# shibatch/rectdetect

Hardware: AMD Instinct MI355X
Metric: 1920x1080 frames/sec (higher is better)
Workload: dtype u8/i32/f32 (bit-exact integer + IEEE f32 stencil path)

## Files before the change

rectdetect_amd/csrc/rd_k_front.hip:

```cpp
#include <stdlib.h>
#include "rd_device.h"
#include "rd_kernels.h"
#include "rectdetect_hip.h"

#define RD_LUT_ATTR __device__
#include "rd_luts.h"

namespace {

using namespace rd;
using namespace rdpix;

struct P3 { float *p[3]; };
struct P3c { const float *p[3]; };
struct SrcZ { const uint8_t *p[RD_ZB_MAX]; };

inline int cdiv(int a, int b) { return (a + b - 1) / b; }
inline dim3 grid2(int iw, int ih) { return dim3(cdiv(iw, 64), cdiv(ih, 4)); }
const dim3 block2(64, 4);
inline int grid1(int n) { int g = cdiv(n, 256); return g < 1 ? 1 : g; }

__device__ __forceinline__ int lerp_lut(const unsigned short *t, int c) { return t[c >> 8] * (256 - (c & 255)) + t[(c >> 8) + 1] * (c & 255); }

__device__ __forceinline__ uint32_t plab_of(const unsigned short *s_s2l, const unsigned short *s_cf, const unsigned short *s_cf2, int b, int g, int r) {
// ... 222 lines not shown
    } else if (FMT == RD_PIX_NV12) yuv_bgr(byte(8 * sr + sx), byte(16 + 2 * j), byte(17 + 2 * j), pb, pg, pr);
    else yuv_bgr(byte(8 * sr + sx), byte(16 + j), byte(20 + j), pb, pg, pr);
    b += pb; g += pg; r += pr;
  }
  b >>= 2; g >>= 2; r >>= 2;
}

template <int FMT>
__global__ __launch_bounds__(256) void k_pix2plab_half_t(uint32_t *__restrict__ out, P3 dst, PixZ src, int iw, int ih, size_t zs) {
  const int z = blockIdx.z;
  const uint8_t *__restrict__ p0 = src.p[0][z], *__restrict__ p1 = src.p[1][z], *__restrict__ p2 = src.p[2][z];
  RD_ZSHIFT(zs, out, dst.p[0], dst.p[1], dst.p[2]);
  __shared__ unsigned short s_s2l[RD_LUT_S2L_N], s_cf[RD_LUT_CF_N], s_cf2[RD_LUT_CF_N];
  __shared__ unsigned short tile[3][64][66];
  const int tid = rd_ty() * 64 + threadIdx.x;
  const int x0 = blockIdx.x * 64, y0 = blockIdx.y * 64;
  const int cx = (tid & 15) * 4, r0 = tid >> 4;
  const int x = x0 + cx, m = min(iw - x, 4);
  uint32_t w[4][HalfW<FMT>::n] = {};
#pragma unroll
  for (int k = 0; k < 4; k++) {
    const int y = y0 + r0 + 16 * k;
    if (m > 0 && y < ih) pix_load_half<FMT>(w[k], p0, p1, p2, src.pitch, x, y, m, src.wide != 0);
  }
  for (int i = tid; i < RD_LUT_S2L_N; i += 256) s_s2l[i] = rd_lut_s2l[i];
  for (int i = tid; i < RD_LUT_CF_N; i += 256) { s_cf[i] = rd_lut_cfunc[i]; s_cf2[i] = rd_lut_cfunc2[i]; }
  __syncthreads();
#pragma unroll
  for (int k = 0; k < 4; k++) {
    const int r = r0 + 16 * k, y = y0 + r;
    if (m <= 0 || y >= ih) continue;
    uint32_t v[4];
#pragma unroll
    for (int j = 0; j < 4; j++) {
      int b, g, rr;
      pix_bgr_half<FMT>(w[k], j, b, g, rr);
      v[j] = plab_of(s_s2l, s_cf, s_cf2, b, g, rr);
      tile[0][r][cx + j] = (unsigned short)(v[j] & 4095u); tile[1][r][cx + j] = (unsigned short)((v[j] >> 12) & 1023u); tile[2][r][cx + j] = (unsigned short)((v[j] >> 22) & 1023u);
    }
    uint32_t *o = out + (size_t)y * iw + x;
    if (m == 4 && (iw & 3) == 0) *(uint4 *)o = make_uint4(v[0], v[1], v[2], v[3]);
    else for (int j = 0; j < m; j++) o[j] = v[j];
  }
  __syncthreads();
  for (int r = rd_ty(); r < 64; r += 4) {
    const int ox = y0 + threadIdx.x, oy = x0 + r;
    if (ox < ih && oy < iw)
      for (int k = 0; k < 3; k++) ((unsigned short *)dst.p[k])[(size_t)oy * ih + ox] = tile[k][threadIdx.x][r];
  }
}

template <typename LD, typename ST> __device__ __forceinline__ void ew4(int n, LD ld, ST st) {
  const int stride = gridDim.x * blockDim.x;
  int i = blockIdx.x * blockDim.x + threadIdx.x;
  for (; i + 3 * stride < n; i += 4 * stride) {
    const auto v0 = ld(i), v1 = ld(i + stride), v2 = ld(i + 2 * stride), v3 = ld(i + 3 * stride);
    st(i, v0); st(i + stride, v1); st(i + 2 * stride, v2); st(i + 3 * stride, v3);
  }
  for (; i < n; i += stride) st(i, ld(i));
}

__global__ void k_unpack_plab(float *__restrict__ L, float *__restrict__ a, float *__restrict__ b, const uint32_t *__restrict__ in, int n) {
  for (int i = blockIdx.x * blockDim.x + threadIdx.x; i < n; i += gridDim.x * blockDim.x) {
    float l, aa, bb;
    unpack_lab(in[i], l, aa, bb);
    L[i] = l; a[i] = aa; b[i] = bb;
  }
}

__global__ void k_pack_plab(uint32_t *__restrict__ out, const float *__restrict__ L, const float *__restrict__ a, const float *__restrict__ b, int n) {
  ew4(n, [=](int i) { return make_float3(L[i], a[i], b[i]); }, [=](int i, float3 v) { out[i] = pack_lab(v.x, v.y, v.z); });
}

template <int MODE>
__global__ __launch_bounds__(256) void k_transpose(P3 dst, P3c src, P3c fwd, P3c bwd, const uint32_t *__restrict__ plab, int np, int W, int H, const int *only_if) {
  if (only_if && *only_if == 0) return;
  __shared__ float tile[3][64][65];
  const int x0 = blockIdx.x * 64, y0 = blockIdx.y * 64;
  for (int r = rd_ty(); r < 64; r += 4) {
    const int x = x0 + threadIdx.x, y = y0 + r;
    if (x < W && y < H) {
      const size_t i = (size_t)y * W + x;
      if (MODE == 1) {
        float l, a, b;
        unpack_lab(plab[i], l, a, b);
        tile[0][r][threadIdx.x] = l; tile[1][r][threadIdx.x] = a; tile[2][r][threadIdx.x] = b;
      } else if (MODE == 2) {
        for (int k = 0; k < np; k++) tile[k][r][threadIdx.x] = bwd.p[k][i] + fwd.p[k][i] - src.p[k][i] * 0.3989422804f;
      } else {
        for (int k = 0; k < np; k++) tile[k][r][threadIdx.x] = src.p[k][i];
      }
    }
  }
  __syncthreads();
  for (int r = rd_ty(); r < 64; r += 4) {
    const int ox = y0 + threadIdx.x, oy = x0 + r;
    if (ox < H && oy < W)
      for (int k = 0; k < np; k++) dst.p[k][(size_t)oy * H + ox] = tile[k][threadIdx.x][r];
  }
}

#define IIR_C0 0.3989422804f
#define IIR_C1 0.1414542400f
#define IIR_C2 -0.0030406818f
#define IIR_C3 -0.0041116157f
#define IIR_C4 0.0006696623f
#define IIR_C5 0.0000498707f
#define IIR_C6 -0.0000449761f
#define IIR_C7 -0.0000051528f
#define IIR_C8 0.2519574622f
#define IIR_C9 -0.0098627835f
#define IIR_C10 -0.0067013653f
#define IIR_C11 0.0012572396f
#define IIR_C12 0.0000481394f
#define IIR_C13 -0.0000097781f
#define IIR_C14 0.0000006462f
#define IIR_WARM 11
#ifndef IIR_CH
#define IIR_CH 16
#endif

#define IF_ROWS_MIN 64
#define IF_WU 32
#define IF_PITCH 65
__host__ __device__ inline int if_nchunks(int H, int rows) {
  int n = (H + rows - 1) / rows;
  if (n > 1 && H % rows != 0 && H % rows < 8) n--;
  return n;
}

typedef float iir_f2 __attribute__((ext_vector_type(2)));
#define IIR_STATE iir_f2 q1 = 0, q2 = 0, q3 = 0, q4 = 0, q5 = 0, q6 = 0, q7 = 0
#define IIR_STEP(i0v)                                                                                                  \
  iir_f2 acc = (iir_f2){IIR_C1, IIR_C8} * q1;                                                                          \
  acc = acc + (iir_f2){IIR_C2, IIR_C9} * q2;                                                                           \
  acc = acc + (iir_f2){IIR_C3, IIR_C10} * q3;                                                                          \
  acc = acc + (iir_f2){IIR_C4, IIR_C11} * q4;                                                                          \
  acc = acc + (iir_f2){IIR_C5, IIR_C12} * q5;                                                                          \
  acc = acc + (iir_f2){IIR_C6, IIR_C13} * q6;                                                                          \
  acc = acc + (iir_f2){IIR_C7, IIR_C14} * q7;                                                                          \
  float d = (i0v) * IIR_C0;                                                                                            \
  d += acc.x;                                                                                                          \
  d += acc.y;
#define IIR_SHIFT(i0v)                                                                                                 \
  q7 = q6; q6 = q5; q5 = q4; q4 = q3; q3 = q2; q2 = q1; q1 = (iir_f2){(i0v), d};

template <int SRC16> struct iir_src { typedef float T; };
template <> struct iir_src<1> { typedef unsigned short T; };
template <int SRC16, typename T> __device__ __forceinline__ float iir_field(T v, float sc, float hf) {
  if (SRC16) return (float)(int)v * sc + hf;
  return (float)v;
}
template <int TOUT, int IF_ROWS, int SRC16>
__global__ __launch_bounds__(128) void k_iir_fused(P3 dst, P3c src, float *__restrict__ tails, int W, int H, int nchunks, int *bad, int np, size_t zs) {
  __shared__ float fwt[(IF_ROWS + 8) * IF_PITCH];
  const int lane = threadIdx.x & 63, anti = threadIdx.x >> 6;
  const int k = blockIdx.y % np, c = blockIdx.z;
  float *dk = k == 0 ? dst.p[0] : (k == 1 ? dst.p[1] : dst.p[2]);
  const float *sk = k == 0 ? src.p[0] : (k == 1 ? src.p[1] : src.p[2]);
  { const size_t rd_zoff_ = (size_t)(blockIdx.y / np) * zs; RD_ZS1(dk); RD_ZS1(sk); RD_ZS1(tails); RD_ZS1(bad); }
  if (blockIdx.x == 0 && k == 0 && blockIdx.z == 0 && threadIdx.x == 0) *bad = 0;
  const int x = blockIdx.x * 64 + lane;
  const bool xin = x < W;
  typedef typename iir_src<SRC16>::T TS;
  const TS *__restrict__ in = (const TS *)sk;
  const unsigned xs = (unsigned)(xin ? x : W - 1) * (unsigned)sizeof(TS), x4 = (unsigned)(xin ? x : W - 1) * 4u;
#define IIR_ROW(ptr) (*(const TS *)((const char *)(ptr) + xs))
#define IIR_OUT(ptr) (*(float *)((char *)(ptr) + x4))
  const float sc = k == 0 ? 1.0f / 4096 : 1.0f / 1024, hf = k == 0 ? 0.5f / 4096 : 0.5f / 1024;
#define IIR_LD(v) iir_field<SRC16>(v, sc, hf)
  const int s0 = c * IF_ROWS, s1 = (c == nchunks - 1) ? H : s0 + IF_ROWS;
  const int mid = s0 + (s1 - s0) / 2;
  float *__restrict__ tl = tails + ((size_t)(k * nchunks + c) * 4 * 7) * W;
  const int ylo = -IIR_WARM, yhi = H + IIR_WARM;
  float cur[IIR_CH], nxt[IIR_CH];
  static_assert(IIR_CH >= 8 && IF_WU % IIR_CH == 0 && (IF_ROWS / 2) % IIR_CH == 0, "the interior path walks whole chunks, half a block per phase");
  if (s0 - IF_WU >= 0 && s1 + IF_WU <= H && s1 - s0 == IF_ROWS) {
#define IIR_CHUNK(PTR, STEP, STORE, TAIL, TIDX) IIR_CHUNK_(PTR, STEP, STORE, TAIL, TIDX, 1)
#define IIR_CHUNK_(PTR, STEP, STORE, TAIL, TIDX, MORE)                                                                  \
    {                                                                                                                    \
      if (MORE) { _Pragma("unroll") for (int j = 0; j < IIR_CH; j++) nxt[j] = IIR_LD(IIR_ROW((PTR) + ((long)(IIR_CH + j) * (STEP)) * W)); } \
      _Pragma("unroll") for (int j = 0; j < IIR_CH; j++) {                                                               \
        IIR_STEP(cur[j]);                                                                                                \
        STORE;                                                                                                           \
        if ((TAIL) >= 0 && j >= IIR_CH - 7 && xin) IIR_OUT(tl + (size_t)((TAIL) * 7 + (TIDX)) * W) = d;                            \
        IIR_SHIFT(cur[j]);                                                                                               \
      }                                                                                                                  \
      _Pragma("unroll") for (int j = 0; j < IIR_CH; j++) cur[j] = nxt[j];                                                \
    }
    constexpr int HALF = IF_ROWS / 2 / IIR_CH;
    IIR_STATE;
    if (!anti) {
      const TS *p = in + (size_t)(s0 - IF_WU) * W;
#pragma unroll
      for (int j = 0; j < IIR_CH; j++) cur[j] = IIR_LD(IIR_ROW(p + (size_t)j * W));
      for (int q = 0; q < IF_WU / IIR_CH - 1; q++) { IIR_CHUNK(p, 1, (void)0, -1, 0); p += (size_t)IIR_CH * W; }
      IIR_CHUNK(p, 1, (void)0, 0, j - (IIR_CH - 7)); p += (size_t)IIR_CH * W;
      float *f = fwt + lane;
      for (int q = 0; q < HALF; q++) { IIR_CHUNK(p, 1, f[j * IF_PITCH] = d, -1, 0); p += (size_t)IIR_CH * W; f += IIR_CH * IF_PITCH; }
      __syncthreads();
      float *o = TOUT ? nullptr : dk + (size_t)mid * W;
#define IIR_FINISH_F { const float r = (f[j * IF_PITCH] + d) - cur[j] * IIR_C0; if (TOUT) f[j * IF_PITCH] = r; else if (xin) IIR_OUT(o + (long)j * W) = r; }
      for (int q = 0; q < HALF - 1; q++) { IIR_CHUNK(p, 1, IIR_FINISH_F, -1, 0); p += (size_t)IIR_CH * W; f += IIR_CH * IF_PITCH; if (!TOUT) o += (size_t)IIR_CH * W; }
      IIR_CHUNK_(p, 1, IIR_FINISH_F, 1, j - (IIR_CH - 7), 0);
#undef IIR_FINISH_F
    } else {
      const TS *p = in + (size_t)(s1 - 1 + IF_WU) * W;
#pragma unroll
      for (int j = 0; j < IIR_CH; j++) cur[j] = IIR_LD(IIR_ROW(p - (long)j * W));
      for (int q = 0; q < IF_WU / IIR_CH - 1; q++) { IIR_CHUNK(p, -1, (void)0, -1, 0); p -= (size_t)IIR_CH * W; }
      IIR_CHUNK(p, -1, (void)0, 2, (IIR_CH - 1) - j); p -= (size_t)IIR_CH * W;
      float *f = fwt + (IF_ROWS - 1) * IF_PITCH + lane;
      for (int q = 0; q < HALF; q++) { IIR_CHUNK(p, -1, f[-j * IF_PITCH] = d, -1, 0); p -= (size_t)IIR_CH * W; f -= IIR_CH * IF_PITCH; }
      __syncthreads();
      float *o = TOUT ? nullptr : dk + (size_t)(mid - 1) * W;
#define IIR_FINISH_B { const float r = d + f[-j * IF_PITCH] - cur[j] * IIR_C0; if (TOUT) f[-j * IF_PITCH] = r; else if (xin) IIR_OUT(o - (long)j * W) = r; }
      for (int q = 0; q < HALF - 1; q++) { IIR_CHUNK(p, -1, IIR_FINISH_B, -1, 0); p -= (size_t)IIR_CH * W; f -= IIR_CH * IF_PITCH; if (!TOUT) o -= (size_t)IIR_CH * W; }
      IIR_CHUNK_(p, -1, IIR_FINISH_B, 3, (IIR_CH - 1) - j, 0);
#undef IIR_FINISH_B
    }
#undef IIR_CHUNK
#undef IIR_CHUNK_
  } else {
    IIR_STATE;
    if (!anti) {
      const int fb = (s0 - IF_WU <= ylo) ? ylo : s0 - IF_WU;
      const int total = s1 - fb;
#pragma unroll
      for (int j = 0; j < IIR_CH; j++) cur[j] = IIR_LD(IIR_ROW(in + (size_t)mirror1(clampi(fb + j, ylo, yhi), H) * W));
      for (int base = 0; base < total; base += IIR_CH) {
#pragma unroll
        for (int j = 0; j < IIR_CH; j++) nxt[j] = IIR_LD(IIR_ROW(in + (size_t)mirror1(clampi(fb + base + IIR_CH + j, ylo, yhi), H) * W));
#pragma unroll
        for (int j = 0; j < IIR_CH; j++) {
          const int yy = fb + base + j;
          if (yy == mid) __syncthreads();
          IIR_STEP(cur[j]);
          if (yy >= s0 && yy < mid) fwt[(yy - s0) * IF_PITCH + lane] = d;
          else if (yy >= mid && yy < s1) {
            const float o = (fwt[(yy - s0) * IF_PITCH + lane] + d) - cur[j] * IIR_C0;
            if (TOUT) fwt[(yy - s0) * IF_PITCH + lane] = o;
            else if (xin) IIR_OUT(dk + (size_t)yy * W) = o;
          }
          if (xin && yy >= s0 - 7 && yy < s0) IIR_OUT(tl + (size_t)(0 * 7 + yy - (s0 - 7)) * W) = d;
          if (xin && yy >= s1 - 7 && yy < s1) IIR_OUT(tl + (size_t)(1 * 7 + yy - (s1 - 7)) * W) = d;
          IIR_SHIFT(cur[j]);
        }
#pragma unroll
        for (int j = 0; j < IIR_CH; j++) cur[j] = nxt[j];
      }
    } else {
      const int bb = (s1 - 1 + IF_WU >= yhi) ? yhi : s1 - 1 + IF_WU;
      const int total = bb - s0 + 1;
#pragma unroll
      for (int j = 0; j < IIR_CH; j++) cur[j] = IIR_LD(IIR_ROW(in + (size_t)mirror1(clampi(bb - j, ylo, yhi), H) * W));
      for (int base = 0; base < total; base += IIR_CH) {
#pragma unroll
        for (int j = 0; j < IIR_CH; j++) nxt[j] = IIR_LD(IIR_ROW(in + (size_t)mirror1(clampi(bb - (base + IIR_CH + j), ylo, yhi), H) * W));
#pragma unroll
        for (int j = 0; j < IIR_CH; j++) {
          const int yy = bb - (base + j);
          if (yy == mid - 1) __syncthreads();
          IIR_STEP(cur[j]);
          if (yy >= mid && yy < s1) fwt[(yy - s0) * IF_PITCH + lane] = d;
          else if (yy >= s0 && yy < mid) {
            const float o = d + fwt[(yy - s0) * IF_PITCH + lane] - cur[j] * IIR_C0;
            if (TOUT) fwt[(yy - s0) * IF_PITCH + lane] = o;
            else if (xin) IIR_OUT(dk + (size_t)yy * W) = o;
          }
          if (xin && yy >= s1 && yy < s1 + 7) IIR_OUT(tl + (size_t)(2 * 7 + yy - s1) * W) = d;
          if (xin && yy >= s0 && yy < s0 + 7) IIR_OUT(tl + (size_t)(3 * 7 + yy - s0) * W) = d;
          IIR_SHIFT(cur[j]);
        }
#pragma unroll
        for (int j = 0; j < IIR_CH; j++) cur[j] = nxt[j];
      }
    }
  }
  if (TOUT) {
    __syncthreads();
    const int rows = s1 - s0;
    for (int col = anti; col < 64; col += 2) {
      const int xx = blockIdx.x * 64 + col;
      if (xx >= W) break;
      float *__restrict__ o = dk + (size_t)xx * H + s0;
      for (int r = lane; r < rows; r += 64) at32(o, (unsigned)r) = fwt[r * IF_PITCH + col];
    }
  }
}

#undef IIR_LD
#undef IIR_ROW
#undef IIR_OUT

#define IC_CH 4
template <int TOUT, int SRC16, int EAGER>
__global__ __launch_bounds__(64 * IC_CH) void k_iir_check_fix(P3 dst, P3c src, P3 fwd, const float *__restrict__ tails, int *bad, int W, int H, int nchunks, int IF_ROWS, int force, int np, size_t zs) {
  const int x = blockIdx.x * 64 + threadIdx.x;
  const int k = blockIdx.y % np, c = blockIdx.z * IC_CH + rd_ty();
  if (c >= nchunks) return;
  float *dk = k == 0 ? dst.p[0] : (k == 1 ? dst.p[1] : dst.p[2]), *fk = k == 0 ? fwd.p[0] : (k == 1 ? fwd.p[1] : fwd.p[2]);
  const float *sk = k == 0 ? src.p[0] : (k == 1 ? src.p[1] : src.p[2]);
  { const size_t rd_zoff_ = (size_t)(blockIdx.y / np) * zs; RD_ZS1(dk); RD_ZS1(sk); RD_ZS1(fk); RD_ZS1(tails); RD_ZS1(bad); }
  if (x >= W) return;
  const int s0 = c * IF_ROWS, s1 = (c == nchunks - 1) ? H : s0 + IF_ROWS;
  const float *me = tails + ((size_t)(k * nchunks + c) * 4 * 7) * W + x;
  bool differ = force != 0 && c == 0;
  const bool chk_f = c > 0 && s0 - IF_WU > -IIR_WARM;
  const bool chk_b = c < nchunks - 1 && s1 - 1 + IF_WU < H + IIR_WARM;
  const float *pv = tails + ((size_t)(k * nchunks + (chk_f ? c - 1 : c)) * 4 * 7) * W + x;
  const float *nx = tails + ((size_t)(k * nchunks + (chk_b ? c + 1 : c)) * 4 * 7) * W + x;
  if (EAGER) {
    unsigned a[14], b[14];
#pragma unroll
    for (int j = 0; j < 7; j++) {
      a[j] = __float_as_uint(me[(size_t)(0 * 7 + j) * W]); b[j] = __float_as_uint(pv[(size_t)(1 * 7 + j) * W]);
      a[7 + j] = __float_as_uint(me[(size_t)(2 * 7 + j) * W]); b[7 + j] = __float_as_uint(nx[(size_t)(3 * 7 + j) * W]);
    }
    unsigned df = 0, db = 0;
#pragma unroll
    for (int j = 0; j < 7; j++) { df |= a[j] ^ b[j]; db |= a[7 + j] ^ b[7 + j]; }
    differ = differ || (chk_f && df != 0) || (chk_b && db != 0);
  } else {
    if (chk_f) {
#pragma unroll
      for (int j = 0; j < 7; j++) differ = differ || (__float_as_uint(me[(size_t)(0 * 7 + j) * W]) != __float_as_uint(pv[(size_t)(1 * 7 + j) * W]));
    }
    if (chk_b) {
#pragma unroll
      for (int j = 0; j < 7; j++) differ = differ || (__float_as_uint(me[(size_t)(2 * 7 + j) * W]) != __float_as_uint(nx[(size_t)(3 * 7 + j) * W]));
    }
  }
  if (!differ) return;
  atomicOr(bad, 1);
  typedef typename iir_src<SRC16>::T TS;
  const TS *__restrict__ in = (const TS *)sk + x;
  const float sc = k == 0 ? 1.0f / 4096 : 1.0f / 1024, hf = k == 0 ? 0.5f / 4096 : 0.5f / 1024;
  float *fw = fk + x;
  {
    IIR_STATE;
    for (int yy = -IIR_WARM; yy < H; yy++) {
      const float i0 = iir_field<SRC16>(in[(size_t)mirror1(yy, H) * W], sc, hf);
      IIR_STEP(i0);
      if (yy >= 0) fw[(size_t)yy * W] = d;
      IIR_SHIFT(i0);
    }
  }
  {
    IIR_STATE;
    for (int yy = H + IIR_WARM; yy >= 0; yy--) {
      const float i0 = iir_field<SRC16>(in[(size_t)mirror1(yy, H) * W], sc, hf);
      IIR_STEP(i0);
      if (yy < H) {
        const float o = d + fw[(size_t)yy * W] - i0 * IIR_C0;
        if (TOUT) dk[(size_t)x * H + yy] = o; else dk[(size_t)yy * W + x] = o;
      }
      IIR_SHIFT(i0);
    }
  }
}

#define RD_IIRCOEF_ATTR __device__ __constant__
#include "rd_iircoef.h"
__global__ __launch_bounds__(128) void k_iir_line(float *dst, const float *__restrict__ src, float *fw, float *bw, int W, int H, int r) {
  const int x = blockIdx.x * 64 + threadIdx.x;
  const bool xin = x < W;
  float C[15];
#pragma unroll
  for (int k = 0; k < 15; k++) C[k] = rd_iircoef[r][k];
  const int warm = r + 1 + 8;
  if (xin) {
    const float *in = src + x;
    float i1 = 0, i2 = 0, i3 = 0, i4 = 0, i5 = 0, i6 = 0, i7 = 0;
    float t0 = 0, t1 = 0, t2 = 0, t3 = 0, t4 = 0, t5 = 0, t6 = 0;
#define IIR_LINE_STEP                                                                                                    \
    const float i0 = in[(size_t)mirror1(yy, H) * W];                                                                     \
    float d = i0 * C[0];                                                                                                 \
    d += C[1] * i1 + C[2] * i2 + C[3] * i3 + C[4] * i4 + C[5] * i5 + C[6] * i6 + C[7] * i7;                              \
    d += C[8] * t0 + C[9] * t1 + C[10] * t2 + C[11] * t3 + C[12] * t4 + C[13] * t5 + C[14] * t6;                         \
    i7 = i6; i6 = i5; i5 = i4; i4 = i3; i3 = i2; i2 = i1; i1 = i0;                                                       \
    t6 = t5; t5 = t4; t4 = t3; t3 = t2; t2 = t1; t1 = t0; t0 = d;
    if (rd_ty() == 0) {
      float *o = fw + x;
      for (int yy = -warm; yy < H; yy++) { IIR_LINE_STEP; if (yy >= 0) o[(size_t)yy * W] = d; }
    } else {
      float *o = bw + x;
      for (int yy = H + warm; yy >= 0; yy--) { IIR_LINE_STEP; if (yy < H) o[(size_t)yy * W] = d; }
    }
#undef IIR_LINE_STEP
  }
  __syncthreads();
  if (!xin) return;
  for (int yy = rd_ty(); yy < H; yy += 2) {
    const size_t p = (size_t)yy * W + x;
    dst[p] = bw[p] + fw[p] - src[p] * C[0];
  }
}

#include "rd_front_helpers.h"

#ifndef EV_PX
#define EV_PX 4
#endif
__device__ __forceinline__ void ev_finish(float2 *__restrict__ dst, int p, float vx, float vy) {
  float len = vx * vx + vy * vy;
  if ((double)len > 1e-10) {
    len = 1.0f / sqrtf(len);
    vx *= len; vy *= len;
  } else {
    vx = vy = 0.70710678118f;
  }
  dst[p] = make_float2(vx, vy);
}
__global__ __launch_bounds__(256) void k_edgevec(float2 *__restrict__ dst, const float *__restrict__ in, int iw, int ih, uint32_t *__restrict__ pack_out, const float *__restrict__ pa, const float *__restrict__ pb, size_t zs) {
  RD_ZSHIFT(zs, dst, in, pack_out, pa, pb);
  const int x = blockIdx.x * 64 + threadIdx.x, y0 = (blockIdx.y * 4 + rd_ty()) * EV_PX;
  if (x >= iw || y0 >= ih) return;
  if (pack_out != nullptr) {
#pragma unroll
    for (int k = 0; k < EV_PX; k++) if (y0 + k < ih) { const int p = (y0 + k) * iw + x; pack_out[p] = pack_lab(in[p], pa[p], pb[p]); }
  }
  const bool interior = blockIdx.x > 0 && blockIdx.y > 0 && (int)(blockIdx.x * 64 + 66) <= iw && (int)((blockIdx.y * 4 + 4) * EV_PX + 2) <= ih;
  if (interior) {
    float w[EV_PX + 4][5];
#pragma unroll
    for (int r = 0; r < EV_PX + 4; r++) {
      const float *row = in + (size_t)(y0 + r - 2) * iw + x;
#pragma unroll
      for (int c = 0; c < 5; c++) w[r][c] = row[c - 2];
    }
#pragma unroll
    for (int k = 0; k < EV_PX; k++) {
      float vx = 0, vy = 0;
#pragma unroll
      for (int yy = -2; yy <= 2; yy++)
#pragma unroll
        for (int xx = -2; xx <= 2; xx++) {
          const float s = w[k + yy + 2][xx + 2];
          vx += v5c((xx + 2) + (yy + 2) * 5) * s;
          vy += v5c((yy + 2) + (xx + 2) * 5) * s;
        }
// ... 176 lines not shown

__device__ __forceinline__ float icfunc(float ft) { return ft > 0.20689270648f ? ft * ft * ft : (ft - 16.0f / 116) * (1.0f / 7.787f); }

__global__ __launch_bounds__(256) void k_plab2bgr(uint8_t *__restrict__ out, const uint32_t *__restrict__ in, int iw, int ih, int ws) {
  const int x = blockIdx.x * 64 + threadIdx.x, y = blockIdx.y * 4 + rd_ty();
  if (x >= iw || y >= ih) return;
  const float xn = 0.950456f, zn = 1.088754f;
  float L, a, b;
  unpack_lab(in[y * iw + x], L, a, b);
  L *= 256; a *= 256; b *= 256;
  float cy;
  if (L > 0.20689270648f) { cy = (L + 16) * (1.0f / 116.0f); cy = cy * cy * cy; }
  else cy = L * (1.0f / 903.3f);
  const float fy = (float)(rd_lut_cfunc[clampi((int)floorf(cy * 1024), 0, 1023)] + 9039) * (1.0f / 65536.0f);
  const float fz = fy - (b - 128) * (1.0f / 200.0f);
  const float fx = fy + (a - 128) * (1.0f / 500.0f);
  const float cx = icfunc(fx) * xn, cz = icfunc(fz) * zn;
  const float r = cx * 3.240479f + cy * -1.537150f + cz * -0.498535f;
  const float g = cx * -0.969256f + cy * 1.875991f + cz * 0.041556f;
  const float bb = cx * 0.055648f + cy * -0.204043f + cz * 1.057311f;
  uint8_t *o = out + (size_t)y * ws + x * 3;
  o[2] = rd_lut_l2s[clampi((int)floorf(r * 1024), 0, 1023)];
  o[1] = rd_lut_l2s[clampi((int)floorf(g * 1024), 0, 1023)];
  o[0] = rd_lut_l2s[clampi((int)floorf(bb * 1024), 0, 1023)];
}

__global__ __launch_bounds__(256) void k_edge_f(float *__restrict__ out, const float *__restrict__ in, int iw, int ih) {
  const int x = blockIdx.x * 64 + threadIdx.x, y = blockIdx.y * 4 + rd_ty();
  if (x >= iw || y >= ih) return;
  const float n = in[mirror2(x, y - 1, iw, ih)], s = in[mirror2(x, y + 1, iw, ih)], w = in[mirror2(x - 1, y, iw, ih)], e = in[mirror2(x + 1, y, iw, ih)];
  float sum = 0, t;
  t = n + w - s - e;
  sum += (in[mirror2(x - 1, y - 1, iw, ih)] - in[mirror2(x + 1, y + 1, iw, ih)]) * t;
  t = n - w + e - s;
  sum += (in[mirror2(x + 1, y - 1, iw, ih)] - in[mirror2(x - 1, y + 1, iw, ih)]) * t;
  out[y * iw + x] = sqrtf(fmaxf(0.0f, sum));
}

__global__ __launch_bounds__(256) void k_edgevec_plab(float2 *__restrict__ dst, const uint32_t *__restrict__ in, int iw, int ih) {
  const int x = blockIdx.x * 64 + threadIdx.x, y = blockIdx.y * 4 + rd_ty();
  if (x >= iw || y >= ih) return;
  float vx3[3] = { 0, 0, 0 }, vy3[3] = { 0, 0, 0 };
#pragma unroll
  for (int yy = -2; yy <= 2; yy++) {
#pragma unroll
    for (int xx = -2; xx <= 2; xx++) {
      float s[3];
      unpack_lab(in[mirror2(x + xx, y + yy, iw, ih)], s[0], s[1], s[2]);
#pragma unroll
      for (int c = 0; c < 3; c++) {
        vx3[c] += v5c((xx + 2) + (yy + 2) * 5) * s[c];
        vy3[c] += v5c((yy + 2) + (xx + 2) * 5) * s[c];
      }
    }
  }
  float l3[3];
#pragma unroll
  for (int c = 0; c < 3; c++) l3[c] = vx3[c] * vx3[c] + vy3[c] * vy3[c];
  float ivlen, vx, vy;
  if (l3[0] >= l3[1] && l3[0] >= l3[2]) { ivlen = l3[0]; vx = vx3[0]; vy = vy3[0]; }
  else if (l3[1] >= l3[2]) { ivlen = l3[1]; vx = vx3[1]; vy = vy3[1]; }
  else { ivlen = l3[2]; vx = vx3[2]; vy = vy3[2]; }
  if ((double)l3[0] >= 1e-6 && (vx3[0] * vx + vy3[0] * vy < 0)) { vx = -vx; vy = -vy; }
  if ((double)ivlen > 1e-10) { ivlen = 1.0f / sqrtf(ivlen); vx *= ivlen; vy *= ivlen; }
  else vx = vy = 0.70710678118f;
  dst[y * iw + x] = make_float2(vx, vy);
}

__global__ __launch_bounds__(256) void k_thincubic(float *__restrict__ out, const float *__restrict__ in, const float2 *__restrict__ vxy, int iw, int ih) {
  const int x = blockIdx.x * 64 + threadIdx.x, y = blockIdx.y * 4 + rd_ty();
  if (x >= iw || y >= ih) return;
  const int p0 = y * iw + x;
  const float2 v = vxy[p0];
  const float am2 = bicubic(in, x - 2 * v.x, y - 2 * v.y, iw, ih);
  const float am1 = bicubic(in, x - 1 * v.x, y - 1 * v.y, iw, ih);
  const float a0 = in[p0];
  const float ap1 = bicubic(in, x + 1 * v.x, y + 1 * v.y, iw, ih);
  const float ap2 = bicubic(in, x + 2 * v.x, y + 2 * v.y, iw, ih);
  const float C = 0.99f;
  out[p0] = (am2 * C <= a0 && am1 * C <= a0 && a0 >= ap1 * C && a0 >= ap2 * C) ? (am2 + am1 + a0 + ap1 + ap2) : 0.0f;
}

}

namespace rdk {

void bgr2plab(hipStream_t s, uint32_t *out, const uint8_t *bgr, int iw, int ih, int ws) {
  hipLaunchKernelGGL(k_bgr2plab, dim3(cdiv(iw, 64), cdiv(ih, 16)), block2, 0, s, out, bgr, iw, ih, ws);
}
void bgr2plab_transposed(hipStream_t s, uint32_t *out, float *const dst[3], const uint8_t *const *bgr, int iw, int ih, int ws, int nz, size_t zs) {
  P3 d = { { dst[0], dst[1], dst[2] } };
  SrcZ z;
  for (int i = 0; i < RD_ZB_MAX; i++) z.p[i] = bgr[i < nz ? i : 0];
  hipLaunchKernelGGL(k_bgr2plab_t, dim3(cdiv(iw, 64), cdiv(ih, 64), nz), block2, 0, s, out, d, z, iw, ih, ws, zs);
}
void bgr2plab_transposed(hipStream_t s, uint32_t *out, float *const dst[3], const uint8_t *bgr, int iw, int ih, int ws) {
  bgr2plab_transposed(s, out, dst, &bgr, iw, ih, ws, 1, 0);
}
static PixZ pixz_of(const uint8_t *const (*planes)[3], const int pitch[3], int nz) {
  PixZ z;
  z.wide = 1;
  for (int k = 0; k < 3; k++) {
    z.pitch[k] = pitch[k];
    if (pitch[k] & 3) z.wide = 0;
    for (int i = 0; i < RD_ZB_MAX; i++) { z.p[k][i] = planes[i < nz ? i : 0][k]; if ((uintptr_t)z.p[k][i] & 3) z.wide = 0; }
  }
  return z;
}
void pix2plab_transposed(hipStream_t s, int fmt, uint32_t *out, float *const dst[3], const uint8_t *const (*planes)[3], const int pitch[3], int iw, int ih, int nz, size_t zs) {
  const P3 d = { { dst[0], dst[1], dst[2] } };
  const PixZ z = pixz_of(planes, pitch, nz);
  const dim3 grid(cdiv(iw, 64), cdiv(ih, 64), nz);
  const bool known = fmt != RD_PIX_BGR && dispatch(fmt, [&](auto f) {
    if constexpr (f.value != RD_PIX_BGR) hipLaunchKernelGGL(k_pix2plab_t<f.value>, grid, block2, 0, s, out, d, z, iw, ih, zs);
  });
  if (!known) abort();
}
void pix2plab_half_transposed(hipStream_t s, int fmt, uint32_t *out, float *const dst[3], const uint8_t *const (*planes)[3], const int pitch[3], int iw, int ih, int nz, size_t zs) {
  const P3 d = { { dst[0], dst[1], dst[2] } };
  const PixZ z = pixz_of(planes, pitch, nz);
  const dim3 grid(cdiv(iw, 64), cdiv(ih, 64), nz);
  if (!dispatch(fmt, [&](auto f) { hipLaunchKernelGGL(k_pix2plab_half_t<f.value>, grid, block2, 0, s, out, d, z, iw, ih, zs); })) abort();
}
void unpack_plab(hipStream_t s, float *L, float *a, float *b, const uint32_t *in, int n) {
  hipLaunchKernelGGL(k_unpack_plab, dim3(ew_grid(n)), dim3(256), 0, s, L, a, b, in, n);
}
void pack_plab(hipStream_t s, uint32_t *out, const float *L, const float *a, const float *b, int n) {
  hipLaunchKernelGGL(k_pack_plab, dim3(ew_grid(n)), dim3(256), 0, s, out, L, a, b, n);
}

static P3 mk3(float *const p[3], int np) { P3 r = { { nullptr, nullptr, nullptr } }; for (int k = 0; k < np; k++) r.p[k] = p[k]; return r; }
static P3c mk3c(const float *const p[3], int np) { P3c r = { { nullptr, nullptr, nullptr } }; for (int k = 0; k < np; k++) r.p[k] = p[k]; return r; }

void transpose_f(hipStream_t s, float *const dst[3], const float *const src[3], int np, int W, int H) {
  P3c z = { { nullptr, nullptr, nullptr } };
  hipLaunchKernelGGL(k_transpose<0>, dim3(cdiv(W, 64), cdiv(H, 64)), block2, 0, s, mk3(dst, np), mk3c(src, np), z, z, (const uint32_t *)nullptr, np, W, H, (const int *)nullptr);
}
static int if_pick_rows(int np, int W, int H, int transpose_out, int nz) {
  (void)np; (void)W; (void)H;
  (void)transpose_out;
#ifndef IF_GROUP_ROWS
#define IF_GROUP_ROWS 128
#endif
  if (nz > 1) return IF_GROUP_ROWS;
  return 64;
}

size_t iir_pass_scratch_floats(int np, int W, int H) { return (size_t)np * if_nchunks(H, IF_ROWS_MIN) * 4 * 7 * W; }

void iir_blur_pass(hipStream_t s, float *const dst[3], const float *const src[3], float *const fwd[3], float *const bwd[3], int np, int W, int H,
                   int transpose_out, float *tails, int *bad, int src16, int nz, size_t zs) {
  const int rows = if_pick_rows(np, W, H, transpose_out, nz);
  const int nchunks = if_nchunks(H, rows);
  const dim3 grid(cdiv(W, 64), np * nz, nchunks);
#define IF_LAUNCH(T, R, S16) hipLaunchKernelGGL((k_iir_fused<T, R, S16>), grid, dim3(128), 0, s, mk3(dst, np), mk3c(src, np), tails, W, H, nchunks, bad, np, zs)
#define IF_LAUNCH_R(R) { if (transpose_out && src16) IF_LAUNCH(1, R, 1); else if (transpose_out) IF_LAUNCH(1, R, 0); else IF_LAUNCH(0, R, 0); }
  switch (rows) {
    case 64: IF_LAUNCH_R(64); break;
    default: IF_LAUNCH_R(128); break;
  }
#undef IF_LAUNCH_R
#undef IF_LAUNCH
  if (nchunks > 1) {
    const dim3 cgrid(grid.x, grid.y, cdiv(nchunks, IC_CH)), cblock(64, IC_CH);
    const int force = getenv("RD_IIR_FORCE_FIX") ? 1 : 0;
#define IC_LAUNCH(T, S16, E) hipLaunchKernelGGL((k_iir_check_fix<T, S16, E>), cgrid, cblock, 0, s, mk3(dst, np), mk3c(src, np), mk3(fwd, np), (const float *)tails, bad, W, H, nchunks, rows, force, np, zs)
    if (nz > 1) { if (transpose_out && src16) IC_LAUNCH(1, 1, 0); else if (transpose_out) IC_LAUNCH(1, 0, 0); else IC_LAUNCH(0, 0, 0); }
    else { if (transpose_out && src16) IC_LAUNCH(1, 1, 1); else if (transpose_out) IC_LAUNCH(1, 0, 1); else IC_LAUNCH(0, 0, 1); }
#undef IC_LAUNCH
  }
  (void)bwd;
}

void iir_blur_lines(hipStream_t s, float *dst, const float *src, float *fw, float *bw, int W, int H, int r) {
  hipLaunchKernelGGL(k_iir_line, dim3(cdiv(W, 64)), dim3(64, 2), 0, s, dst, src, fw, bw, W, H, r);
}

void convert_bgr_lumaf(hipStream_t s, uint8_t *out, const float *in, float f, int iw, int ih, int ws) {
  hipLaunchKernelGGL(k_convert_bgr_lumaf, grid2(iw, ih), block2, 0, s, out, in, f, iw, ih, ws);
}
void convert_bgr_labeli(hipStream_t s, uint8_t *out, const int *in, int bgc, int iw, int ih, int ws) {
  hipLaunchKernelGGL(k_convert_bgr_labeli, grid2(iw, ih), block2, 0, s, out, in, bgc, iw, ih, ws);
}
void plab2bgr(hipStream_t s, uint8_t *out, const uint32_t *in, int iw, int ih, int ws) {
  hipLaunchKernelGGL(k_plab2bgr, grid2(iw, ih), block2, 0, s, out, in, iw, ih, ws);
}
void edge_f(hipStream_t s, float *out, const float *in, int iw, int ih) {
  hipLaunchKernelGGL(k_edge_f, grid2(iw, ih), block2, 0, s, out, in, iw, ih);
}
void edgevec_plab(hipStream_t s, float *vxy, const uint32_t *in, int iw, int ih) {
  hipLaunchKernelGGL(k_edgevec_plab, grid2(iw, ih), block2, 0, s, (float2 *)vxy, in, iw, ih);
}
void thincubic(hipStream_t s, float *out, const float *in, const float *vxy, int iw, int ih) {
  hipLaunchKernelGGL(k_thincubic, grid2(iw, ih), block2, 0, s, out, in, (const float2 *)vxy, iw, ih);
}
void edgevec(hipStream_t s, float *vxy, const float *in, int iw, int ih, uint32_t *pack_out, const float *a, const float *b, int nz, size_t zs) {
  hipLaunchKernelGGL(k_edgevec, dim3(cdiv(iw, 64), cdiv(ih, 4 * EV_PX), nz), block2, 0, s, (float2 *)vxy, in, iw, ih, pack_out, a, b, zs);
}
void edge_plab(hipStream_t s, float *out, const uint32_t *in, int iw, int ih, int nz, size_t zs) {
  hipLaunchKernelGGL(k_edge_plab, dim3(cdiv(iw, 64), cdiv(ih, 4 * EP_PX), nz), block2, 0, s, out, in, iw, ih, zs);
}
void thinthres(hipStream_t s, float *out, const float *in, const float *vxy, int iw, int ih, int nz, size_t zs) {
  hipLaunchKernelGGL(k_thinthres, dim3(cdiv(iw, 64), cdiv(ih, TT_ROWS), nz), dim3(64, 4), 0, s, out, in, (const float2 *)vxy, iw, ih, zs);
}
void threshold_f(hipStream_t s, float *out, const float *in, float lo, float thr, float hi, int n) {
  hipLaunchKernelGGL(k_threshold_f, dim3(ew_grid(n)), dim3(256), 0, s, out, in, lo, thr, hi, n);
}
void threshold_i(hipStream_t s, int *out, const int *in, int lo, int thr, int hi, int n) {
  hipLaunchKernelGGL(k_threshold_i, dim3(ew_grid(n)), dim3(256), 0, s, out, in, lo, thr, hi, n);
}
void cast_i_f(hipStream_t s, int *out, const float *in, float scale, int n) {
  hipLaunchKernelGGL(k_cast_i_f, dim3(ew_grid(n)), dim3(256), 0, s, out, in, scale, n);
}
void cast_c_i(hipStream_t s, int8_t *out, const int *in, int n) {
  hipLaunchKernelGGL(k_cast_c_i, dim3(ew_grid(n)), dim3(256), 0, s, out, in, n);
}
void clear_i(hipStream_t s, int *out, int n) {
  if (n > 0) hipLaunchKernelGGL(k_clear_i, dim3(ew_grid(n)), dim3(256), 0, s, out, n);
}
void copy_i(hipStream_t s, int *out, const int *in, int n) {
  if (n > 0) hipLaunchKernelGGL(k_copy_i, dim3(ew_grid(n)), dim3(256), 0, s, out, in, n);
}
void rand_i(hipStream_t s, int *out, uint64_t seed, int n) {
  if (n > 0) hipLaunchKernelGGL(k_rand_i, dim3(ew_grid(n)), dim3(256), 0, s, out, seed, n);
}

}
```

Measured before the change: 3380.

## Split IIR blur into full-chunk and edge kernels, park forward results in registers

The interior IIR kernel is rewritten. Forward partial results now stay in registers instead of shared memory, and the two waves swap their filter state through a small LDS buffer at the midpoint. Transposed output goes through a per-wave staging tile flushed in batches. Loads use larger chunks with scalar base pointers, and ragged last chunks go to a separate edge kernel launched after the main one. This aims to cut LDS traffic and branching in the common path, at the cost of high register pressure (HALF-sized park array), one extra launch, and a more complex store pattern.

```diff
diff --git a/rectdetect_amd/csrc/rd_k_front.hip b/rectdetect_amd/csrc/rd_k_front.hip
--- a/rectdetect_amd/csrc/rd_k_front.hip
+++ b/rectdetect_amd/csrc/rd_k_front.hip
@@ -398,14 +398,14 @@
   return (float)v;
 }
 template <int TOUT, int IF_ROWS, int SRC16>
-__global__ __launch_bounds__(128) void k_iir_fused(P3 dst, P3c src, float *__restrict__ tails, int W, int H, int nchunks, int *bad, int np, size_t zs) {
+__global__ __launch_bounds__(128) void k_iir_fused_edge(P3 dst, P3c src, float *__restrict__ tails, int W, int H, int nchunks, int nf, int *bad, int np, size_t zs) {
   __shared__ float fwt[(IF_ROWS + 8) * IF_PITCH];
   const int lane = threadIdx.x & 63, anti = threadIdx.x >> 6;
-  const int k = blockIdx.y % np, c = blockIdx.z;
+  const int k = blockIdx.y % np, c = nf + (int)blockIdx.z;
   float *dk = k == 0 ? dst.p[0] : (k == 1 ? dst.p[1] : dst.p[2]);
   const float *sk = k == 0 ? src.p[0] : (k == 1 ? src.p[1] : src.p[2]);
   { const size_t rd_zoff_ = (size_t)(blockIdx.y / np) * zs; RD_ZS1(dk); RD_ZS1(sk); RD_ZS1(tails); RD_ZS1(bad); }
-  if (blockIdx.x == 0 && k == 0 && blockIdx.z == 0 && threadIdx.x == 0) *bad = 0;
+  if (blockIdx.x == 0 && k == 0 && c == 0 && threadIdx.x == 0) *bad = 0;
   const int x = blockIdx.x * 64 + lane;
   const bool xin = x < W;
   typedef typename iir_src<SRC16>::T TS;
@@ -420,54 +420,7 @@
   float *__restrict__ tl = tails + ((size_t)(k * nchunks + c) * 4 * 7) * W;
   const int ylo = -IIR_WARM, yhi = H + IIR_WARM;
   float cur[IIR_CH], nxt[IIR_CH];
-  static_assert(IIR_CH >= 8 && IF_WU % IIR_CH == 0 && (IF_ROWS / 2) % IIR_CH == 0, "the interior path walks whole chunks, half a block per phase");
-  if (s0 - IF_WU >= 0 && s1 + IF_WU <= H && s1 - s0 == IF_ROWS) {
-#define IIR_CHUNK(PTR, STEP, STORE, TAIL, TIDX) IIR_CHUNK_(PTR, STEP, STORE, TAIL, TIDX, 1)
-#define IIR_CHUNK_(PTR, STEP, STORE, TAIL, TIDX, MORE)                                                                  \
-    {                                                                                                                    \
-      if (MORE) { _Pragma("unroll") for (int j = 0; j < IIR_CH; j++) nxt[j] = IIR_LD(IIR_ROW((PTR) + ((long)(IIR_CH + j) * (STEP)) * W)); } \
-      _Pragma("unroll") for (int j = 0; j < IIR_CH; j++) {                                                               \
-        IIR_STEP(cur[j]);                                                                                                \
-        STORE;                                                                                                           \
-        if ((TAIL) >= 0 && j >= IIR_CH - 7 && xin) IIR_OUT(tl + (size_t)((TAIL) * 7 + (TIDX)) * W) = d;                            \
-        IIR_SHIFT(cur[j]);                                                                                               \
-      }                                                                                                                  \
-      _Pragma("unroll") for (int j = 0; j < IIR_CH; j++) cur[j] = nxt[j];                                                \
-    }
-    constexpr int HALF = IF_ROWS / 2 / IIR_CH;
-    IIR_STATE;
-    if (!anti) {
-      const TS *p = in + (size_t)(s0 - IF_WU) * W;
-#pragma unroll
-      for (int j = 0; j < IIR_CH; j++) cur[j] = IIR_LD(IIR_ROW(p + (size_t)j * W));
-      for (int q = 0; q < IF_WU / IIR_CH - 1; q++) { IIR_CHUNK(p, 1, (void)0, -1, 0); p += (size_t)IIR_CH * W; }
-      IIR_CHUNK(p, 1, (void)0, 0, j - (IIR_CH - 7)); p += (size_t)IIR_CH * W;
-      float *f = fwt + lane;
-      for (int q = 0; q < HALF; q++) { IIR_CHUNK(p, 1, f[j * IF_PITCH] = d, -1, 0); p += (size_t)IIR_CH * W; f += IIR_CH * IF_PITCH; }
-      __syncthreads();
-      float *o = TOUT ? nullptr : dk + (size_t)mid * W;
-#define IIR_FINISH_F { const float r = (f[j * IF_PITCH] + d) - cur[j] * IIR_C0; if (TOUT) f[j * IF_PITCH] = r; else if (xin) IIR_OUT(o + (long)j * W) = r; }
-      for (int q = 0; q < HALF - 1; q++) { IIR_CHUNK(p, 1, IIR_FINISH_F, -1, 0); p += (size_t)IIR_CH * W; f += IIR_CH * IF_PITCH; if (!TOUT) o += (size_t)IIR_CH * W; }
-      IIR_CHUNK_(p, 1, IIR_FINISH_F, 1, j - (IIR_CH - 7), 0);
-#undef IIR_FINISH_F
-    } else {
-      const TS *p = in + (size_t)(s1 - 1 + IF_WU) * W;
-#pragma unroll
-      for (int j = 0; j < IIR_CH; j++) cur[j] = IIR_LD(IIR_ROW(p - (long)j * W));
-      for (int q = 0; q < IF_WU / IIR_CH - 1; q++) { IIR_CHUNK(p, -1, (void)0, -1, 0); p -= (size_t)IIR_CH * W; }
-      IIR_CHUNK(p, -1, (void)0, 2, (IIR_CH - 1) - j); p -= (size_t)IIR_CH * W;
-      float *f = fwt + (IF_ROWS - 1) * IF_PITCH + lane;
-      for (int q = 0; q < HALF; q++) { IIR_CHUNK(p, -1, f[-j * IF_PITCH] = d, -1, 0); p -= (size_t)IIR_CH * W; f -= IIR_CH * IF_PITCH; }
-      __syncthreads();
-      float *o = TOUT ? nullptr : dk + (size_t)(mid - 1) * W;
-#define IIR_FINISH_B { const float r = d + f[-j * IF_PITCH] - cur[j] * IIR_C0; if (TOUT) f[-j * IF_PITCH] = r; else if (xin) IIR_OUT(o - (long)j * W) = r; }
-      for (int q = 0; q < HALF - 1; q++) { IIR_CHUNK(p, -1, IIR_FINISH_B, -1, 0); p -= (size_t)IIR_CH * W; f -= IIR_CH * IF_PITCH; if (!TOUT) o -= (size_t)IIR_CH * W; }
-      IIR_CHUNK_(p, -1, IIR_FINISH_B, 3, (IIR_CH - 1) - j, 0);
-#undef IIR_FINISH_B
-    }
-#undef IIR_CHUNK
-#undef IIR_CHUNK_
-  } else {
+  {
     IIR_STATE;
     if (!anti) {
       const int fb = (s0 - IF_WU <= ylo) ? ylo : s0 - IF_WU;
@@ -533,6 +486,137 @@
       for (int r = lane; r < rows; r += 64) at32(o, (unsigned)r) = fwt[r * IF_PITCH + col];
     }
   }
+}
+
+__device__ __forceinline__ unsigned iir_off(unsigned o) { asm("" : "+v"(o)); return o; }
+template <typename T> __device__ __forceinline__ __attribute__((address_space(1))) T *iir_uni(T *p) {
+  __attribute__((address_space(1))) T *g = (__attribute__((address_space(1))) T *)p;
+  asm("" : "+s"(g));
+  return g;
+}
+#ifndef IIR_PCH
+#define IIR_PCH 16
+#endif
+#ifndef IF_TB
+#define IF_TB 32
+#endif
+#define IF_TP (64 + 64 / IF_TB)
+#ifdef IF_WPE
+#define IF_WPE_ATTR __attribute__((amdgpu_waves_per_eu(IF_WPE)))
+#else
+#define IF_WPE_ATTR
+#endif
+template <int TOUT, int IF_ROWS, int SRC16>
+__global__ __launch_bounds__(128) IF_WPE_ATTR void k_iir_fused(P3 dst, P3c src, float *__restrict__ tails, int W, int H, int nchunks, int *bad, int np, size_t zs) {
+  constexpr int HALF = IF_ROWS / 2, CH = IIR_PCH, CPI = 64 / IF_TB;
+  static_assert(CH >= 8 && IF_WU % CH == 0 && HALF % CH == 0 && HALF % IF_TB == 0 && 64 % IF_TB == 0, "whole chunks and whole batches, half a block per phase");
+  __shared__ float swp[2 * 14 * 64];
+  __shared__ float stg[TOUT ? 2 * IF_TB * IF_TP : 1];
+  const int lane = threadIdx.x & 63, anti = __builtin_amdgcn_readfirstlane((int)(threadIdx.x >> 6));
+  const int fz = __builtin_amdgcn_readfirstlane((int)(blockIdx.y / np)), k = blockIdx.y - fz * np, c = blockIdx.z;
+  float *dk = k == 0 ? dst.p[0] : (k == 1 ? dst.p[1] : dst.p[2]);
+  const float *sk = k == 0 ? src.p[0] : (k == 1 ? src.p[1] : src.p[2]);
+  { const size_t rd_zoff_ = (size_t)fz * zs; RD_ZS1(dk); RD_ZS1(sk); RD_ZS1(tails); RD_ZS1(bad); }
+  if (blockIdx.x == 0 && k == 0 && blockIdx.z == 0 && threadIdx.x == 0) *bad = 0;
+  const int x = blockIdx.x * 64 + lane;
+  const bool xin = x < W;
+  typedef typename iir_src<SRC16>::T TS;
+  const TS *__restrict__ in = (const TS *)sk;
+  const unsigned xs = (unsigned)(xin ? x : W - 1) * (unsigned)sizeof(TS), x4 = (unsigned)(xin ? x : W - 1) * 4u;
+#undef IIR_ROW
+#undef IIR_OUT
+#define IIR_ROW(ptr) (*(const TS *)((const char *)(ptr) + xo_))
+#define IIR_OUT(ptr) (*(float *)((char *)(ptr) + iir_off(x4)))
+  const float sc = k == 0 ? 1.0f / 4096 : 1.0f / 1024, hf = k == 0 ? 0.5f / 4096 : 0.5f / 1024;
+  const int s0 = c * IF_ROWS, s1 = s0 + IF_ROWS, mid = s0 + HALF;
+  float *__restrict__ tl = tails + ((size_t)(k * nchunks + c) * 4 * 7) * W;
+  const long rs = anti ? -(long)W : (long)W;
+  float cur[CH], nxt[CH], park[HALF];
+#define IIR_PSTEPS(...)                                                                                                  \
+      _Pragma("unroll") for (int j = 0; j < CH; j++) {                                                                   \
+        IIR_STEP(cur[j]);                                                                                                \
+        __VA_ARGS__;                                                                                                     \
+        IIR_SHIFT(cur[j]);                                                                                               \
+      }                                                                                                                  \
+      _Pragma("unroll") for (int j = 0; j < CH; j++) cur[j] = nxt[j];
+#define IIR_PCHUNK(MORE, NEXT, NSTEP, ...)                                                                               \
+    {                                                                                                                    \
+      if (MORE) { const TS *n_ = (NEXT); const unsigned xo_ = iir_off(xs); _Pragma("unroll") for (int j = 0; j < CH; j++) { nxt[j] = IIR_LD(IIR_ROW(iir_uni(n_))); n_ += (NSTEP); } } \
+      IIR_PSTEPS(__VA_ARGS__)                                                                                            \
+    }
+#define IIR_PARK(dst, v) asm("v_mov_b32 %0, %1" : "=v"(dst) : "v"(v))
+  IIR_STATE;
+  const TS *p = in + (size_t)(anti ? s1 - 1 : s0) * W;
+  const TS *const pb = in + (size_t)(anti ? mid : mid - 1) * W;
+  float *const tw = tl + (size_t)(anti ? 2 * 7 + 6 : 0) * W;
+#define IIR_WTAIL if (j >= CH - 7 && xin) IIR_OUT(iir_uni(tw + (long)(j - (CH - 7)) * rs)) = d
+  if (anti ? s1 + IF_WU <= H : s0 - IF_WU >= 0) {
+    const TS *w = p - IF_WU * rs;
+    { const unsigned xo_ = iir_off(xs);
+#pragma unroll
+      for (int j = 0; j < CH; j++) cur[j] = IIR_LD(IIR_ROW(iir_uni(w + (long)j * rs))); }
+    for (int q = 0; q < IF_WU / CH - 1; q++) { IIR_PCHUNK(1, w + CH * rs, rs, (void)0); w += CH * rs; }
+    IIR_PCHUNK(1, p, rs, IIR_WTAIL);
+  } else {
+    const int dy = anti ? -1 : 1, y0 = anti ? s1 - 1 + IF_WU : s0 - IF_WU;
+    const unsigned xo_ = iir_off(xs);
+    auto eld = [&](int yy) -> float {
+      const int yc = clampi(yy, -IIR_WARM, H + IIR_WARM);
+      const float v = IIR_LD(IIR_ROW(iir_uni(in + (size_t)mirror1(yc, H) * W)));
+      return yy == yc ? v : 0.0f;
+    };
+#define IIR_PCHUNK_E(YN, ...) { _Pragma("unroll") for (int j = 0; j < CH; j++) nxt[j] = eld((YN) + j * dy); IIR_PSTEPS(__VA_ARGS__) }
+#pragma unroll
+    for (int j = 0; j < CH; j++) cur[j] = eld(y0 + j * dy);
+    for (int q = 0; q < IF_WU / CH - 1; q++) IIR_PCHUNK_E(y0 + (q + 1) * CH * dy, (void)0)
+    IIR_PCHUNK(1, p, rs, IIR_WTAIL);
+  }
+#undef IIR_WTAIL
+#pragma unroll
+  for (int q = 0; q < HALF / CH; q++) {
+    const bool last = q == HALF / CH - 1;
+    IIR_PCHUNK(1, last ? pb : p + CH * rs, last ? -rs : rs, IIR_PARK(park[q * CH + j], d)); p += CH * rs;
+  }
+  {
+    float *mine = swp + anti * (14 * 64) + lane, *theirs = swp + (anti ^ 1) * (14 * 64) + lane;
+#define IIR_SWAP(n, q) mine[(2 * n) * 64] = q.x; mine[(2 * n + 1) * 64] = q.y;
+    IIR_SWAP(0, q1) IIR_SWAP(1, q2) IIR_SWAP(2, q3) IIR_SWAP(3, q4) IIR_SWAP(4, q5) IIR_SWAP(5, q6) IIR_SWAP(6, q7)
+#undef IIR_SWAP
+    __syncthreads();
+#define IIR_SWAP(n, q) q.x = theirs[(2 * n) * 64]; q.y = theirs[(2 * n + 1) * 64];
+    IIR_SWAP(0, q1) IIR_SWAP(1, q2) IIR_SWAP(2, q3) IIR_SWAP(3, q4) IIR_SWAP(4, q5) IIR_SWAP(5, q6) IIR_SWAP(6, q7)
+#undef IIR_SWAP
+  }
+  p = pb;
+  float *const tt = tl + (size_t)(anti ? 1 * 7 : 3 * 7 + 6) * W;
+  float *o = dk + (size_t)(anti ? mid : mid - 1) * W;
+  float *const st = stg + (TOUT ? anti * (IF_TB * IF_TP) : 0);
+  const int br = lane % IF_TB, bc = lane / IF_TB;
+  const float *const sl = st + (anti ? br : IF_TB - 1 - br) * IF_TP + bc;
+  const unsigned bo = ((unsigned)bc * (unsigned)H + (unsigned)br) * 4u;
+#pragma unroll
+  for (int q = 0; q < HALF / CH; q++) {
+    const bool last = q == HALF / CH - 1;
+    IIR_PCHUNK(!last, p - CH * rs, -rs, {
+      const int i = q * CH + j;
+      const float r = (park[HALF - 1 - i] + d) - cur[j] * IIR_C0;
+      if (TOUT) st[(i % IF_TB) * IF_TP + lane] = r; else if (xin) IIR_OUT(iir_uni(o - (long)j * rs)) = r;
+      if (i >= HALF - 7 && xin) IIR_OUT(iir_uni(tt - (long)(i - (HALF - 7)) * rs)) = d;
+      if (TOUT && i % IF_TB == IF_TB - 1) {
+        __builtin_amdgcn_fence(__ATOMIC_RELEASE, "wavefront"); __builtin_amdgcn_wave_barrier(); __builtin_amdgcn_fence(__ATOMIC_ACQUIRE, "wavefront");
+        const int lowest = anti ? mid + (i / IF_TB) * IF_TB : mid - (i / IF_TB + 1) * IF_TB;
+        float *const ob = dk + (size_t)(blockIdx.x * 64) * H + lowest;
+        _Pragma("unroll") for (int n = 0; n < IF_TB; n++)
+          if ((int)blockIdx.x * 64 + n * CPI + bc < W) *(float *)((char *)iir_uni(ob + (size_t)(n * CPI) * H) + bo) = sl[n * CPI];
+        __builtin_amdgcn_fence(__ATOMIC_RELEASE, "wavefront"); __builtin_amdgcn_wave_barrier(); __builtin_amdgcn_fence(__ATOMIC_ACQUIRE, "wavefront");
+      }
+    });
+    p -= CH * rs; if (!TOUT) o -= CH * rs;
+  }
+#undef IIR_PCHUNK
+#undef IIR_PCHUNK_E
+#undef IIR_PSTEPS
+#undef IIR_PARK
 }
 
 #undef IIR_LD
@@ -1015,11 +1099,17 @@
                    int transpose_out, float *tails, int *bad, int src16, int nz, size_t zs) {
   const int rows = if_pick_rows(np, W, H, transpose_out, nz);
   const int nchunks = if_nchunks(H, rows);
+  const int nf = (H - (nchunks - 1) * rows == rows) ? nchunks : nchunks - 1;
   const dim3 grid(cdiv(W, 64), np * nz, nchunks);
-#define IF_LAUNCH(T, R, S16) hipLaunchKernelGGL((k_iir_fused<T, R, S16>), grid, dim3(128), 0, s, mk3(dst, np), mk3c(src, np), tails, W, H, nchunks, bad, np, zs)
-#define IF_LAUNCH_R(R) { if (transpose_out && src16) IF_LAUNCH(1, R, 1); else if (transpose_out) IF_LAUNCH(1, R, 0); else IF_LAUNCH(0, R, 0); }
+  const dim3 fgrid(grid.x, grid.y, nf), egrid(grid.x, grid.y, nchunks - nf);
+#define IF_LAUNCH(T, R, S16) { if (nf > 0) hipLaunchKernelGGL((k_iir_fused<T, R, S16>), fgrid, dim3(128), 0, s, mk3(dst, np), mk3c(src, np), tails, W, H, nchunks, bad, np, zs); \
+    if (nf < nchunks) hipLaunchKernelGGL((k_iir_fused_edge<T, R, S16>), egrid, dim3(128), 0, s, mk3(dst, np), mk3c(src, np), tails, W, H, nchunks, nf, bad, np, zs); }
+#define IF_LAUNCH_R(R) { if (transpose_out && src16) IF_LAUNCH(1, R, 1) else if (transpose_out) IF_LAUNCH(1, R, 0) else IF_LAUNCH(0, R, 0) }
   switch (rows) {
     case 64: IF_LAUNCH_R(64); break;
+#if IF_GROUP_ROWS != 64 && IF_GROUP_ROWS != 128
+    case IF_GROUP_ROWS: IF_LAUNCH_R(IF_GROUP_ROWS); break;
+#endif
     default: IF_LAUNCH_R(128); break;
   }
 #undef IF_LAUNCH_R
```

After: 3463, median of 6. 1.02x the previous value.
